# DarylFernandes99/custom-yolo-implmentation

Measured on AMD Instinct MI355X. Metric: images/sec (640x640 bf16), higher is better.
Workload: dtype bf16; 1 GPU; preset s (width 32..512, depth 1) 640x640 train step (fwd+DFL/QFL loss+bwd+grad sync+AdamW), COCO-80 synthetic, 32 img/GPU; global_batch=32, parallelism=dp1, hip_graph=True, optimizer_in_graph=True, deterministic_mode=False

## Files before the change

custom-yolo-implmentation_amd/csrc/conv_halo.hip:

```cpp
#include "conv_dev.h"

namespace {

constexpr int HROW = 48;
constexpr int HW = 18;

template <typename T, int TH, int BN, bool ACC>
__global__ __launch_bounds__((TH / 4) * (BN / 64) * 64) void k_conv_halo(GeomDev g, const T* __restrict__ src,
                                                                        const T* __restrict__ wm,
                                                                        const float* __restrict__ bias,
                                                                        T* __restrict__ dst, int tiles_h, int tiles_w,
                                                                        int ntile_n) {
    constexpr int WGM = TH / 4, WGN = BN / 64, NTHR = WGM * WGN * 64;
    constexpr int HH = TH + 2, HPX = HH * HW;
    constexpr int HR = (HPX * 4 + NTHR - 1) / NTHR;
    constexpr int WR = (BN * 4) / NTHR;
    static_assert((BN * 4) % NTHR == 0 && WR >= 1, "weight tile must divide over the workgroup");
    using ops = mfma_ops<T>;
    using frag = typename ops::frag;
    __shared__ __attribute__((aligned(16))) T halo[2][HPX * HROW];
    __shared__ __attribute__((aligned(16))) T wl[2][BN][LDSROW];

    const int tid = threadIdx.x, lane = tid & 63, wave = tid >> 6;
    const BlockTile bt = block_tile<TH, 16, BN>(tiles_h, tiles_w, ntile_n);
    const int n = bt.n, y0 = bt.y0, x0 = bt.x0, cd0 = bt.cd0;

    const int shift = (g.Ws + 1) * g.lds;
    const __amdgpu_buffer_rsrc_t rsa = __builtin_amdgcn_make_buffer_rsrc(const_cast<T*>(src) - shift, 0, (g.N * g.Hs * g.Ws * g.lds + shift) * 2, BUF_FLAGS);
    const __amdgpu_buffer_rsrc_t rsb = __builtin_amdgcn_make_buffer_rsrc(const_cast<T*>(wm), 0, g.e.Cd * g.Kpad * 2, BUF_FLAGS);
    int hvoff[HR], hlds[HR];
#pragma unroll
    for (int r = 0; r < HR; ++r) {
        const int h = tid + NTHR * r;
        const int px = h >> 2, ck = h & 3;
        const int hy = px / HW, hx = px - hy * HW;
        const bool ok = h < HPX * 4 && (unsigned)(y0 - 1 + hy) < (unsigned)g.Hs && (unsigned)(x0 - 1 + hx) < (unsigned)g.Ws;
        hvoff[r] = ok ? ((hy * g.Ws + hx) * g.lds + ck * 8) * 2 : BUF_OOB;
        hlds[r] = h < HPX * 4 ? px * HROW + ck * 8 : -1;
    }
    const int hsoff0 = (((n * g.Hs + y0 - 1) * g.Ws + x0 - 1) * g.lds + shift) * 2;
    const int kseg = tid & 3, wrow0 = tid >> 2;
    const int sk = (kseg ^ ((-(wrow0 >> 2)) & 3)) * 8;
    int wvoff[WR];
#pragma unroll
    for (int i = 0; i < WR; ++i) {
        const int row = wrow0 + i * (NTHR / 4);
        wvoff[i] = (cd0 + row < g.e.Cd) ? ((cd0 + row) * g.Kpad + kseg * 8) * 2 : BUF_OOB;
    }

    uint4 rh[HR], rw[WR];
    auto load_halo = [&](int chunk) {
#pragma unroll
        for (int r = 0; r < HR; ++r) {
            const u32x4 v = __builtin_amdgcn_raw_buffer_load_b128(rsa, hvoff[r], hsoff0 + chunk * 64, 0);
            rh[r] = make_uint4(v.x, v.y, v.z, v.w);
        }
    };
    auto store_halo = [&](int buf) {
#pragma unroll
        for (int r = 0; r < HR; ++r)
            if (hlds[r] >= 0) *reinterpret_cast<uint4*>(&halo[buf][hlds[r]]) = rh[r];
    };
    auto load_w = [&](int wcol) {
#pragma unroll
        for (int i = 0; i < WR; ++i) {
            const u32x4 v = __builtin_amdgcn_raw_buffer_load_b128(rsb, wvoff[i], wcol * 2, 0);
            rw[i] = make_uint4(v.x, v.y, v.z, v.w);
        }
    };
    auto store_w = [&](int buf) {
#pragma unroll
        for (int i = 0; i < WR; ++i) *reinterpret_cast<uint4*>(&wl[buf][wrow0 + i * (NTHR / 4)][sk]) = rw[i];
    };

    const int wgm = wave / WGN, wgn = wave - wgm * WGN;
    const int crow = wgn * 64;
    const int fr = lane & 15, fg = lane >> 4;
    const int fk = (fg ^ ((-(fr >> 2)) & 3)) * 8;
    int abase[4];
#pragma unroll
    for (int i = 0; i < 4; ++i) abase[i] = ((wgm * 4 + i + 1) * HW + fr + 1) * HROW + fg * 8;
    f32x4 acc[4][4];
#pragma unroll
    for (int i = 0; i < 4; ++i)
#pragma unroll
        for (int j = 0; j < 4; ++j) acc[i][j] = (f32x4){0.f, 0.f, 0.f, 0.f};

    const int nchunk = g.Cs / BK;
    load_halo(0);
    load_w(0);
    store_halo(0);
    store_w(0);
    __syncthreads();
    int tap = 0, chunk = 0, it = 0;
    const int nit = nchunk * g.ntaps;
    for (; it < nit; ++it) {
        const int wb = it & 1, hb = chunk & 1;
        int ntap = tap + 1, nchk = chunk;
        if (ntap == g.ntaps) { ntap = 0; ++nchk; }
        const bool more = it + 1 < nit;
        const bool new_halo = more && ntap == 0;
        if (more) load_w(ntap * g.Cs + nchk * BK);
        if (new_halo) load_halo(nchk);
        const int toff = (((int)((g.dh_pack >> (2 * tap)) & 3u) - 1) * HW + ((int)((g.dw_pack >> (2 * tap)) & 3u) - 1)) * HROW;
        frag fa[4], fb[4];
#pragma unroll
        for (int j = 0; j < 4; ++j) fa[j] = *reinterpret_cast<const frag*>(&wl[wb][crow + j * 16 + fr][fk]);
#pragma unroll
        for (int i = 0; i < 4; ++i) fb[i] = *reinterpret_cast<const frag*>(&halo[hb][abase[i] + toff]);
#pragma unroll
        for (int i = 0; i < 4; ++i)
#pragma unroll
            for (int j = 0; j < 4; ++j) acc[i][j] = ops::mma(fa[j], fb[i], acc[i][j]);
        if (more) store_w(wb ^ 1);
        if (new_halo) store_halo(hb ^ 1);
        __syncthreads();
        tap = ntap;
        chunk = nchk;
    }

    const int cq = fg * 4;
    float bv[4][4];
    bias_blocks<4>(bias, cd0 + crow, cq, g.e, bv);
    const int ox = x0 + fr;
#pragma unroll
    for (int i = 0; i < 4; ++i) {
        const int oy = y0 + wgm * 4 + i;
        const bool pv = oy < g.Hg && ox < g.Wg;
        store_pixel_blocks<T, 4, ACC>(g.e, acc[i], bv, dst, pv ? ((long)n * g.Hd + oy) * (long)g.Wd + ox : 0, pv, cd0 + crow, cq, lane);
        if (!pv) {
#pragma unroll
            for (int j = 0; j < 4; ++j) acc[i][j] = (f32x4){0.f, 0.f, 0.f, 0.f};
        }
    }

    if (g.e.stats != nullptr)
        conv_stats_epilogue<T, 4, 4>(acc, reinterpret_cast<float*>(&wl[0][0][0]), BN, g.e.stats, cd0, g.e.Cd, crow, cq, fr, tid, NTHR);
}

template <typename T, int TH, int BN>
void launch_halo(const GeomDev& d, const void* src, const void* wm, const float* bias, void* dst, int accumulate,
                 hipStream_t st) {
    constexpr int NTHR = (TH / 4) * (BN / 64) * 64;
    const int th = (d.Hg + TH - 1) / TH, tw = (d.Wg + 15) / 16, tn = (d.e.Cd + BN - 1) / BN;
    const dim3 grid((unsigned)(d.N * th * tw * tn));
    with_acc(accumulate, [&](auto acc) {
        hipLaunchKernelGGL((k_conv_halo<T, TH, BN, decltype(acc)::value>), grid, dim3(NTHR), 0, st, d, (const T*)src, (const T*)wm,
                           bias, (T*)dst, th, tw, tn);
    });
}

}

int halo_conv_eligible(const ConvGeom& g) {
    return g.sstride == 1 && g.ostep == 1 && g.ooff_h == 0 && g.ooff_w == 0 && g.ntaps > 1 && g.Cs % 32 == 0 && g.Cd >= 64 &&
           g.Hg == g.Hs && g.Wg == g.Ws && g.Hd == g.Hg && g.Wd == g.Wg;
}

int halo_conv_launch(const ConvGeom& g, int variant, const void* src, const void* wm, const float* bias, void* dst,
                     int accumulate, int dtype, hipStream_t st) {
    const GeomDev d = to_dev(g);
#define HALO_T(T_)                                                                              \
    switch (variant) {                                                                          \
        case 1: launch_halo<T_, 8, 128>(d, src, wm, bias, dst, accumulate, st); break;          \
        case 2: launch_halo<T_, 16, 128>(d, src, wm, bias, dst, accumulate, st); break;         \
        case 3: launch_halo<T_, 16, 64>(d, src, wm, bias, dst, accumulate, st); break;          \
        default: launch_halo<T_, 8, 64>(d, src, wm, bias, dst, accumulate, st); break;          \
    }
    if (dtype == YOLO_BF16) { HALO_T(bf16_t) } else { HALO_T(f16_t) }
#undef HALO_T
    return YOLO_LAUNCH_CHECK();
}
```

custom-yolo-implmentation_amd/csrc/conv_host.h:

```cpp
#pragma once
#include "common.h"
#include "conv_geom.h"

enum ConvKind {
    CONV_NONE = -1,
    CONV_VALU = 0,
    CONV_GATHER = 1,
    CONV_HALO = 2,
    CONV_RING = 3,
    CONV_ROWS = 4,
    CONV_UP2 = 5
};
struct RingTile { int bm, bn, nst, bk; };
struct ConvChoice {
    int kind;
    int joint;
    int variant;
    int bn;
    RingTile ring;
};
ConvChoice conv_select(const ConvGeom* gs, int n, int cls, int dtype, const void* src, const void* wm, const void* dst, int algo);

ConvTune& conv_tune();
int conv_wide_flag();

static inline bool desc_addressable(long elems) { return elems < (1L << 30); }
static inline bool pixels_addressable(long npix) { return npix < (1L << 31); }

int mfma_conv_addressable(const ConvGeom& g, int dtype, const void* src, const void* wm, const void* dst);

int valu_conv_launch(const ConvGeom& g, const void* src, const void* wm, const float* bias, void* dst, int accumulate, int dtype,
                     hipStream_t st);
int mfma_conv_eligible(const ConvGeom& g, int dtype, const void* src, const void* wm, const void* dst);
int mfma_conv_launch(const ConvGeom& g, int bn, const void* src, const void* wm, const float* bias, void* dst, int accumulate,
                     int dtype, hipStream_t st);
int halo_conv_eligible(const ConvGeom& g);
int halo_conv_launch(const ConvGeom& g, int variant, const void* src, const void* wm, const float* bias, void* dst,
                     int accumulate, int dtype, hipStream_t st);
int ring_conv_eligible(const ConvGeom& g, int dtype, const void* src, const void* wm, const void* dst);
int ring_conv_launch(const ConvGeom* gs, int n, const RingTile& t, const long* wm_off, long wm_elems, const void* src,
                     const void* wm, const float* bias, void* dst, int accumulate, int dtype, hipStream_t st);
int rows_conv_eligible(const ConvGeom& g);
int rows_conv_launch(const ConvGeom& g, int variant, const void* src, const void* wm, const float* bias, void* dst, int accumulate,
                     int dtype, hipStream_t st);
int up2_conv_eligible(const ConvGeom* gs, int dtype);
int up2_conv_launch(const ConvGeom* gs, int variant, const long* wm_off, long wm_elems, const void* src, const void* wm, void* dst,
                    int accumulate, int dtype, hipStream_t st);
int f32_conv_eligible(const ConvGeom& g, const void* src, const void* wm, const void* dst);
int f32_conv_launch(const ConvGeom& g, const float* src, const float* wm, const float* bias, float* dst, int accumulate,
                    hipStream_t st);

int f32_wgrad_eligible(const void* x, int ldx, const void* dy, int ldy, int Cin, int Cout);
int f32_wgrad_launch(const float* x, int ldx, const float* dy, int ldy, float* dwp, int Kpad, int N, int H, int W, int Cin,
                     int OH, int OW, int Cout, int k, int stride, hipStream_t st);
int mfma_wgrad_eligible(int Cin, int Cout, int ldx, int ldy, int dtype, const void* x, const void* dy);
int mfma_wgrad_launch(const void* x, int ldx, const void* dy, int ldy, float* dwp, int Kpad, int N, int H, int W,
                      int Cin, int OH, int OW, int Cout, int k, int stride, int dtype, hipStream_t st);
long mfma_wgrad2_plan(int Kpad, int N, int H, int W, int Cin, int OH, int OW, int Cout, int k);
long mfma_wgrad2_ws_elems(int Kpad, int N, int H, int W, int Cin, int OH, int OW, int Cout, int k);
int mfma_wgrad2_launch(const void* x, int ldx, const void* dy, int ldy, float* part, void* dw_oihw, int dw_dtype, int Kpad,
                       int N, int H, int W, int Cin, int OH, int OW, int Cout, int k, int stride, int dtype, hipStream_t st);

struct DwPlan {
    int cvb, ncy;
    int ncol, ncb;
    int wg;
    int hb, nb, grid;
    int hb_wg, nb_wg, grid_wg;
};
DwPlan dw_plan(int N, int H, int W, int C);
int dw_tune_set(int variant);
bool dw_takes_rows(int N, int H, int W, int C, bool wgrad);
int dw16_launch(bool flip, const void* x, int ldx, const float* w, void* y, int ldy, int N, int H, int W, int C, int dtype,
                int accumulate, float* stats, hipStream_t st, const float* bias = nullptr, int act = 0);
int dw16_wgrad_launch(const void* x, int ldx, const void* dy, int ldy, float* partial, int nslab, int* nrows, int N, int H, int W,
                      int C, int dtype, hipStream_t st);

extern "C" int yolo_bn_stats_acc(const void* y, int ldy, long npix, int C, int dtype, float* acc, hipStream_t st);
extern "C" int yolo_copy_channels(const void* src, int ld_src, void* dst, int ld_dst, long npix, int C, int accumulate, int dtype,
                                  hipStream_t st);

static inline bool conv_supported(int k, int stride) { return (k == 1 && stride == 1) || (k == 3 && (stride == 1 || stride == 2)); }
static inline bool conv_supported(int k, int stride, int Cin, int Cout) {
    return conv_supported(k, stride) && Cin >= 0 && Cout >= 0 && (long)k * k * (Cin > Cout ? Cin : Cout) <= 2147483647L - 31;
}
```

custom-yolo-implmentation_amd/csrc/conv_rows.hip:

```cpp
#include "conv_dev.h"

namespace {

template <typename T, int W, int WGM, int NWAVE, int WN, int NST, bool ACC>
__global__ __launch_bounds__(64 * NWAVE) void k_conv_rows(GeomDev g, const T* __restrict__ src, const T* __restrict__ wm,
                                                   const float* __restrict__ bias, T* __restrict__ dst, int tiles_h,
                                                   int tiles_w, int ntile_n) {
    constexpr int R = WGM * 80 / W, HWID = W == 16 ? 18 : W + 8, HH = R + 2, HPX = HH * HWID;
    constexpr int WGN = NWAVE / WGM;
    constexpr int NTHR = 64 * NWAVE, BN = WGN * WN * 16;
    constexpr int HP = ((HPX + 15) / 16 + NWAVE - 1) / NWAVE;
    constexpr int DW = (3 * BN / 16 + NWAVE - 1) / NWAVE;
    constexpr int HBUF = NWAVE * HP * 1024, STAGE = NWAVE * DW * 1024;
    static_assert(R * W == WGM * 80 && NST >= 3 && NST <= 4 && NWAVE == 4, "block shape");
    using ops = mfma_ops<T>;
    using frag = typename ops::frag;
    extern __shared__ __attribute__((aligned(1024))) char rows_smem[];
    const unsigned lds0 = __builtin_amdgcn_readfirstlane((unsigned)(size_t)(__attribute__((address_space(3))) char*)rows_smem);

    const int tid = threadIdx.x, lane = tid & 63, wave = __builtin_amdgcn_readfirstlane(tid >> 6);
    const BlockTile bt = block_tile<R, W, BN>(tiles_h, tiles_w, ntile_n);
    const int n = bt.n, y0 = bt.y0, x0 = bt.x0, cd0 = bt.cd0;

    const int shift = (g.Ws + 1) * g.lds;
    const int a_bytes = (g.N * g.Hs * g.Ws * g.lds + shift) * 2, w_bytes = g.e.Cd * g.Kpad * 2;
    int hvoff[HP], wvoff[DW];
#pragma unroll
    for (int i = 0; i < HP; ++i) {
        const int px = (wave * HP + i) * 16 + (lane >> 2), ck = (lane & 3) ^ ((px >> 1) & 3);
        const int hy = px / HWID, hx = px - hy * HWID;
        const bool ok = px < HPX && (unsigned)(y0 - 1 + hy) < (unsigned)g.Hs && (unsigned)(x0 + hx - 1) < (unsigned)g.Ws;
        hvoff[i] = (ok && ck * 8 < g.Cs) ? ((hy * g.Ws + hx) * g.lds + ck * 8) * 2 : BUF_OOB;
    }
    const int hsoff0 = (((n * g.Hs + y0 - 1) * g.Ws + x0 - 1) * g.lds + shift) * 2;
#pragma unroll
    for (int j = 0; j < DW; ++j) {
        const int rs = (wave * DW + j) * 16 + (lane >> 2);
        const int tl = rs / BN, row = rs - tl * BN;
        const int kseg = (lane & 3) ^ ((-(row >> 2)) & 3);
        wvoff[j] = (tl < 3 && cd0 + row < g.e.Cd && kseg * 8 < g.Cs) ? ((cd0 + row) * g.Kpad + tl * g.Cs + kseg * 8) * 2 : BUF_OOB;
    }
    const int nchunk = (g.Cs + BK - 1) / BK, nit = nchunk * 3;
    auto issue_halo = [&](int chunk) {
        const __amdgpu_buffer_rsrc_t rsa = __builtin_amdgcn_make_buffer_rsrc(const_cast<T*>(src) - shift, 0, chunk < nchunk ? a_bytes : 0, BUF_FLAGS);
        const unsigned base = lds0 + (chunk & 1) * HBUF + wave * (HP * 1024);
#pragma unroll
        for (int i = 0; i < HP; ++i) lds_dma_piece(rsa, base + i * 1024, hvoff[i], hsoff0 + chunk * 64);
    };
    int wstep = 0, wchunk = 0, wrow = 0, wbuf = 0;
    auto issue_w = [&]() {
        const __amdgpu_buffer_rsrc_t rsb = __builtin_amdgcn_make_buffer_rsrc(const_cast<T*>(wm), 0, wstep < nit ? w_bytes : 0, BUF_FLAGS);
        const unsigned base = lds0 + 2 * HBUF + wbuf * STAGE + wave * (DW * 1024);
        const int soff = (3 * wrow * g.Cs + wchunk * BK) * 2;
#pragma unroll
        for (int j = 0; j < DW; ++j) lds_dma_piece(rsb, base + j * 1024, wvoff[j], soff);
        ++wstep;
        if (++wrow == 3) { wrow = 0; ++wchunk; }
        if (++wbuf == NST) wbuf = 0;
    };

    const int wgm = wave / WGN, wgn = wave - wgm * WGN;
    const int crow = wgn * WN * 16;
    const int fr = lane & 15, fg = lane >> 4;
    const int fk = (fg ^ ((-(fr >> 2)) & 3)) * 16;
    int aoff[5][9];
#pragma unroll
    for (int i = 0; i < 5; ++i) {
        const int p = (wgm * 5 + i) * 16 + fr, pr = p / W, pc = p - pr * W;
#pragma unroll
        for (int tap = 0; tap < 9; ++tap) {
            const int px = (pr + (int)((g.dh_pack >> (2 * tap)) & 3u)) * HWID + pc + (int)((g.dw_pack >> (2 * tap)) & 3u);
            aoff[i][tap] = px * 64 + ((fg ^ ((px >> 1) & 3)) << 4);
        }
    }
    const int woff = (crow + fr) * 64 + fk;
    f32x4 acc[5][WN];
#pragma unroll
    for (int i = 0; i < 5; ++i)
#pragma unroll
        for (int j = 0; j < WN; ++j) acc[i][j] = (f32x4){0.f, 0.f, 0.f, 0.f};

    issue_halo(0);
#pragma unroll
    for (int s = 0; s < NST - 1; ++s) issue_w();
    int rbuf = 0;
    auto step = [&](auto srow_c, auto par_c, int chunk) {
        constexpr int srow = decltype(srow_c)::value, par = decltype(par_c)::value;
        constexpr bool patch_newer = srow != 0 && (NST == 4 || srow == 1);
        dma_wait<(NST - 2) * DW + (patch_newer ? HP : 0)>();
        __builtin_amdgcn_s_barrier();
        if (srow == 0) issue_halo(chunk + 1);
        issue_w();
        const char* hp = rows_smem + par * HBUF;
        const char* wp = rows_smem + 2 * HBUF + (NST == 3 ? srow : rbuf) * STAGE;
#pragma unroll
        for (int tl = 0; tl < 3; ++tl) {
            const int tap = 3 * srow + tl;
            frag fa[WN], fb[5];
#pragma unroll
            for (int j = 0; j < WN; ++j) fa[j] = *reinterpret_cast<const frag*>(wp + (tl * BN + j * 16) * 64 + woff);
#pragma unroll
            for (int i = 0; i < 5; ++i) fb[i] = *reinterpret_cast<const frag*>(hp + aoff[i][tap]);
#pragma unroll
            for (int i = 0; i < 5; ++i)
#pragma unroll
                for (int j = 0; j < WN; ++j) acc[i][j] = ops::mma(fa[j], fb[i], acc[i][j]);
        }
        if (++rbuf == NST) rbuf = 0;
    };
    using c0 = ic<0>; using c1 = ic<1>; using c2 = ic<2>;
    int chunk = 0;
    for (; chunk + 1 < nchunk; chunk += 2) {
        step(c0{}, c0{}, chunk); step(c1{}, c0{}, chunk); step(c2{}, c0{}, chunk);
        step(c0{}, c1{}, chunk + 1); step(c1{}, c1{}, chunk + 1); step(c2{}, c1{}, chunk + 1);
    }
    if (chunk < nchunk) { step(c0{}, c0{}, chunk); step(c1{}, c0{}, chunk); step(c2{}, c0{}, chunk); }
    dma_wait<0>();
    __syncthreads();

    const int cq = fg * 4;
    float bv[WN][4];
    bias_blocks<WN>(bias, cd0 + crow, cq, g.e, bv);
#pragma unroll
    for (int i = 0; i < 5; ++i) {
        const int p = (wgm * 5 + i) * 16 + fr, pr = p / W, pc = p - pr * W;
        const int oy = y0 + pr, ox = x0 + pc;
        const bool live = oy < g.Hg && ox < g.Wg;
        store_pixel_blocks<T, WN, ACC>(g.e, acc[i], bv, dst, live ? ((long)n * g.Hd + oy) * (long)g.Wd + ox : 0, live, cd0 + crow, cq, lane);
        if (!live) {
#pragma unroll
            for (int j = 0; j < WN; ++j) acc[i][j] = (f32x4){0.f, 0.f, 0.f, 0.f};
        }
    }

    if (g.e.stats != nullptr)
        conv_stats_epilogue<T, 5, WN>(acc, reinterpret_cast<float*>(rows_smem), BN, g.e.stats, cd0, g.e.Cd, crow, cq, fr, tid, NTHR);
}

template <typename T, int W, int WGM, int NWAVE, int WN, int NST>
int launch_rows(const GeomDev& d, const void* src, const void* wm, const float* bias, void* dst, int accumulate, hipStream_t st) {
    constexpr int R = WGM * 80 / W, BN = (NWAVE / WGM) * WN * 16, HPX = (R + 2) * (W == 16 ? 18 : W + 8);
    constexpr size_t lds = 2 * (size_t)(NWAVE * (((HPX + 15) / 16 + NWAVE - 1) / NWAVE)) * 1024 + (size_t)NST * NWAVE * ((3 * BN / 16 + NWAVE - 1) / NWAVE) * 1024;
    const int th = (d.Hg + R - 1) / R, tw = W == 16 ? (d.Wg + 15) / 16 : 1, tn = (d.e.Cd + BN - 1) / BN;
    const dim3 grid((unsigned)(d.N * th * tw * tn));
    return with_acc(accumulate, [&](auto acc) {
        return launch_dyn_lds<k_conv_rows<T, W, WGM, NWAVE, WN, NST, decltype(acc)::value>>(grid, dim3(64 * NWAVE), lds, st, d, (const T*)src,
                                                                                            (const T*)wm, bias, (T*)dst, th, tw, tn);
    });
}

}

int rows_conv_eligible(const ConvGeom& g) {
    if (!(g.sstride == 1 && g.ostep == 1 && g.ooff_h == 0 && g.ooff_w == 0 && g.ntaps == 9 && (g.Cs % 32 == 0 || g.Cs == 16) && g.Cd >= 16 &&
          g.Cd % 8 == 0 && g.Hg == g.Hs && g.Wg == g.Ws && g.Hd == g.Hg && g.Wd == g.Wg))
        return 0;
    for (int t = 0; t < 9; ++t)
        if (g.dh[t] < -1 || g.dh[t] > 1 || g.dw[t] < -1 || g.dw[t] > 1) return 0;
    if (g.Cd < 64 || g.Cs == 16) return 3;
    return (g.Wg == 20 || g.Wg == 40) ? 1 : 2;
}

int rows_conv_launch(const ConvGeom& g, int variant, const void* src, const void* wm, const float* bias, void* dst, int accumulate,
                     int dtype, hipStream_t st) {
    const GeomDev d = to_dev(g);
#define ROWS_W(T_, W_)                                                                                               \
    switch (variant) {                                                                                               \
        case 2: return launch_rows<T_, W_, 1, 4, 2, 3>(d, src, wm, bias, dst, accumulate, st);                          \
        case 3: return launch_rows<T_, W_, 1, 4, 1, 3>(d, src, wm, bias, dst, accumulate, st);                       \
        case 4: return launch_rows<T_, W_, 2, 4, 2, 3>(d, src, wm, bias, dst, accumulate, st);                       \
        default: return launch_rows<T_, W_, 1, 4, 1, 4>(d, src, wm, bias, dst, accumulate, st);                         \
    }
#define ROWS_T(T_)                                                                                                   \
    if (variant == 6) return launch_rows<T_, 16, 2, 4, 2, 3>(d, src, wm, bias, dst, accumulate, st);    \
    if (variant == 7) return launch_rows<T_, 16, 4, 4, 2, 3>(d, src, wm, bias, dst, accumulate, st);    \
    if (g.Wg == 20) { ROWS_W(T_, 20) }                                                                               \
    ROWS_W(T_, 40)
    if (dtype == YOLO_BF16) { ROWS_T(bf16_t) }
    ROWS_T(f16_t)
#undef ROWS_T
#undef ROWS_W
}
```

include/yolo_hip.h:

```cpp
#ifndef YOLO_HIP_H
#define YOLO_HIP_H
#include <stddef.h>
#include <stdint.h>

#ifdef __cplusplus
extern "C" {
#endif

#ifndef __HIP__
typedef struct ihipStream_t* hipStream_t;
#endif

#define YOLO_F32 0
#define YOLO_BF16 1
#define YOLO_F16 2
#define YOLO_ERR_ARG 1001
#define YOLO_ERR_DTYPE 1002
#define YOLO_ACT_IDENTITY 0
#define YOLO_ACT_SILU 1

long yolo_abi_hash(void);

int yolo_memset0(void* p, size_t bytes, hipStream_t st);
int yolo_ncm_to_nhwc(const void* src, int src_dtype, long sn, long sc, long off, void* dst, int dst_dtype, int ld, int N, int C, int HW, hipStream_t st);
int yolo_nhwc_to_ncm(const void* src, int src_dtype, int ld, void* dst, int dst_dtype, long sn, long sc, long off, int N, int C, int HW, hipStream_t st);
int yolo_head_group(int pack, int n, void* const* branches, const int* lds, const int* Cs, const int* HWs, const int* c_offs, const int* m_offs, void* preds, int cp, int M, int N, int dtype, hipStream_t st);
int yolo_copy_channels(const void* src, int ld_src, void* dst, int ld_dst, long npix, int C, int accumulate, int dtype, hipStream_t st);
int yolo_scale_inplace(void* x, long n, int dtype, const float* scale_dev, hipStream_t st);
int yolo_add_n(const void* s0, int ld0, const void* s1, int ld1, const void* s2, int ld2, const void* s3, int ld3, int nsrc, void* dst, int ld_dst, long npix, int C, int dtype, hipStream_t st);

int yolo_conv_kpad(int O, int I, int k, int stride, int mode, int cls);
long yolo_conv_dgrad_wbuf_elems(int O, int I, int k, int stride);
int yolo_conv_pack_weights(const void* w_oihw, int w_dtype, int O, int I, int k, int stride, int mode, void* out, int out_dtype, hipStream_t st);
int yolo_conv_unpack_wgrad(const float* dwp, int O, int I, int k, void* dw_oihw, int dw_dtype, hipStream_t st);
int yolo_pack_job_bytes();
int yolo_pack_job_count(int stride, int mode);
long yolo_pack_job_fill(void* jobs_host, const void* w, int w_dtype, void* out, int out_elem_bytes, int O, int I, int k, int stride, int mode, long start);
long yolo_pack_jobs_finalize(void* jobs_host, int njobs);
int yolo_pack_batched(const void* jobs_dev, int njobs, long nchunks, int out_dtype, hipStream_t st);
int yolo_adamw_job_bytes();
int yolo_adamw_job_fill(void* jobs_host, int index, void* p, int p_dtype, const void* g, int g_dtype, float* m, float* v, long n);
long yolo_adamw_jobs_finalize(void* jobs_host, int njobs);
int yolo_adamw_jobs_set_grads(void* jobs_host, int njobs, const void* const* grads);
int yolo_adamw_step(const void* jobs_dev, int njobs, long nchunks, const double* hyper, float* step, const float* grad_scale, const float* found_inf, hipStream_t st);
int yolo_adamw_job_set_ema(void* jobs_host, int index, float* ema, double* ema_ctl);
int yolo_ema_lerp(const void* jobs_dev, int njobs, long nchunks, const double* ema_ctl, const float* skip_flag, hipStream_t st);
int yolo_adamw_amp_step(const void* jobs_dev, int njobs, long nchunks, const double* hyper, float* step, float* amp_state, int* growth_tracker, float growth_factor, float backoff_factor, int growth_interval, hipStream_t st);
int yolo_grad_sqnorm(const void* jobs_dev, int njobs, long nchunks, float* partials, float* found_inf, hipStream_t st);
int yolo_grad_clip_finalize(const float* partials, long nparts, float* clip_state, const float* grad_scale, hipStream_t st);
int yolo_adamw_clip_step(const void* jobs_dev, int njobs, long nchunks, const double* hyper, float* step, const float* grad_scale, const float* found_inf, const float* clip_state, hipStream_t st);
int yolo_amp_update_scale(float* amp_state, int* growth_tracker, float growth_factor, float backoff_factor, int growth_interval, hipStream_t st);
int yolo_sgd_step(const void* jobs_dev, int njobs, long nchunks, const double* hyper, float* step, const float* grad_scale, const float* found_inf, const float* clip_state, hipStream_t st);
int yolo_sgd_amp_step(const void* jobs_dev, int njobs, long nchunks, const double* hyper, float* step, float* amp_state, int* growth_tracker, float growth_factor, float backoff_factor, int growth_interval, hipStream_t st);
int yolo_copy_job_bytes();
int yolo_copy_job_fill(void* jobs_host, int index, const void* src, int src_dtype, void* dst, int dst_dtype, long n);
long yolo_copy_jobs_finalize(void* jobs_host, int njobs);
int yolo_multi_copy(const void* jobs_dev, int njobs, long nchunks, float scale, hipStream_t st);
int yolo_conv2d_fwd(const void* x, int ldx, const void* wp, const float* bias, void* y, int ldy, float* stats_acc, int N, int H, int W, int Cin, int OH, int OW, int Cout, int k, int stride, int dtype, int algo, hipStream_t st);
int yolo_conv2d_fwd_act(const void* x, int ldx, const void* wp, const float* bias, const void* res, int ldr, void* y, int ldy, int N, int H, int W, int Cin, int OH, int OW, int Cout, int k, int stride, int act, int dtype, hipStream_t st);
int yolo_conv2d_dgrad(const void* dy, int lddy, const void* wb, void* dx, int lddx, int N, int H, int W, int Cin, int OH, int OW, int Cout, int k, int stride, int accumulate, int dtype, int algo, hipStream_t st);
int yolo_conv2d_dgrad_acc2(const void* dy, int lddy, const void* wb, void* dx, int lddx, const void* acc2, int ld2, int N, int H, int W, int Cin, int OH, int OW, int Cout, int k, int stride, int dtype, int algo, hipStream_t st);
long yolo_conv2d_wgrad_ws_elems(const void* x, int ldx, const void* dy, int ldy, int N, int H, int W, int Cin, int OH, int OW, int Cout, int k, int stride, int dtype, int algo);
int yolo_conv2d_wgrad(const void* x, int ldx, const void* dy, int ldy, float* ws, void* dw_oihw, int dw_dtype, int N, int H, int W, int Cin, int OH, int OW, int Cout, int k, int stride, int dtype, int algo, hipStream_t st);
int yolo_conv_tune_set(int bn, int tap_inner, int halo, int dma, int ring, int bm, int nst, int bk);
int yolo_wgrad_tune_set(int to, int ti, int blocks, int min_per);
int yolo_wgrad_tune_pf(int pf);
int yolo_conv_wide_set(int on);
int yolo_conv2d_plan(int N, int H, int W, int Cin, int OH, int OW, int Cout, int k, int stride, int mode, int cls, int dtype);
long yolo_conv2d_wgrad_plan(int N, int H, int W, int Cin, int OH, int OW, int Cout, int k, int stride, int dtype);
int yolo_stem_im2col(const void* img, int img_dtype, void* col, int col_dtype, int N, int H, int W, int OH, int OW, hipStream_t st);
int yolo_stem_pack_weights(const void* w, int w_dtype, int Cout, void* out, int out_dtype, hipStream_t st);
int yolo_stem_unpack_wgrad(const float* dw32, int Cout, void* dw, int dw_dtype, hipStream_t st);
int yolo_stem_conv_eligible(int img_dtype, int dtype, int Cout);
int yolo_stem_conv_fwd(const float* img, const void* wp, void* y, int ldy, float* stats, int N, int H, int W, int OH, int OW, int Cout, const float* bias, int act, int dtype, hipStream_t st);
int yolo_stem_wgrad_slabs();
int yolo_stem_wgrad(const float* img, const void* dy, int ldy, float* partial, void* dw, int dw_dtype, int N, int H, int W, int OH, int OW, int Cout, int dtype, hipStream_t st);
long yolo_stem_bn_wgrad_ws_elems(int Cout);
int yolo_stem_bn_wgrad(const float* img, const void* dout, int ldd, const void* y, int ldy, const float* scale, const float* shift, const void* gamma, const float* mean, const float* invstd, float* partial, void* dw, int dw_dtype, void* dgamma, void* dbeta, int N, int H, int W, int OH, int OW, int Cout, int act, int dtype, int pdt, hipStream_t st);
int yolo_dwconv3x3_fwd(const void* x, int ldx, const float* w, void* y, int ldy, int N, int H, int W, int C, int dtype, hipStream_t st);
int yolo_dwconv3x3_fwd_stats(const void* x, int ldx, const float* w, void* y, int ldy, float* stats, int N, int H, int W, int C, int dtype, hipStream_t st);
int yolo_dwconv3x3_fwd_act(const void* x, int ldx, const float* w, const float* bias, void* y, int ldy, int N, int H, int W, int C, int act, int dtype, hipStream_t st);
int yolo_dwconv3x3_dgrad(const void* dy, int lddy, const float* w, void* dx, int lddx, int N, int H, int W, int C, int accumulate, int dtype, hipStream_t st);
int yolo_dw_wgrad_nslab(int N, int H);
int yolo_dwconv3x3_wgrad(const void* x, int ldx, const void* dy, int ldy, float* dw, float* partial, int N, int H, int W, int C, int dtype, hipStream_t st);
int yolo_dw_tune_set(int variant);
int yolo_dw_plan(int N, int H, int W, int C, int field);

int yolo_reduce_nblk(long npix, int C);
int yolo_bn_stats(const void* y, int ldy, long npix, int C, int dtype, float* partial, int nblk, hipStream_t st);
int yolo_bn_finalize(const float* partial, int nblk, long count, int C, const void* gamma, const void* beta, void* running_mean, void* running_var, float momentum, float eps, float* mean, float* invstd, float* scale, float* shift, int pdtype, int bdtype, hipStream_t st);
int yolo_bn_eval_coeffs(const void* gamma, const void* beta, const void* running_mean, const void* running_var, float eps, int C, float* scale, float* shift, int pdtype, int bdtype, hipStream_t st);
int yolo_sum_finalize(const float* partial, int nblk, int C, float* out, hipStream_t st);
int yolo_bn_act_fwd(const void* y, int ldy, const float* scale, const float* shift, const void* res, int ldres, void* out, int ldout, long npix, int C, int act, int dtype, hipStream_t st);
int yolo_bn_act_bwd_reduce(const void* dout, int ldd, const void* y, int ldy, const float* scale, const float* shift, const float* mean, const float* invstd, long npix, int C, int act, int dtype, float* partial, int nblk, hipStream_t st);
int yolo_bn_bwd_finalize(const float* partial, int nblk, long count, int C, const void* gamma, const float* mean, const float* invstd, void* dgamma, void* dbeta, float* coef, int pdtype, hipStream_t st);
int yolo_bn_act_bwd_apply(const void* dout, int ldd, const void* y, int ldy, const float* scale, const float* shift, const float* mean, const float* invstd, const float* coef, void* dy, int lddy, long npix, int C, int act, int dtype, hipStream_t st);
int yolo_bn_acc_elems(int C);
int yolo_bn_stats_acc(const void* y, int ldy, long npix, int C, int dtype, float* acc, hipStream_t st);
int yolo_bn_finalize_acc(const float* acc, long count, int C, const void* gamma, const void* beta, void* running_mean, void* running_var, float momentum, float eps, float* mean, float* invstd, float* scale, float* shift, int pdtype, int bdtype, hipStream_t st);
int yolo_bn_act_fwd_train(const void* y, int ldy, const float* acc, long count, const void* gamma, const void* beta, void* running_mean, void* running_var, float momentum, float eps, float* mean, float* invstd, float* scale, float* shift, const void* res, int ldres, void* out, int ldout, long npix, int C, int act, int dtype, int pdtype, int bdtype, hipStream_t st);
int yolo_bn_bwd_reduce_acc(const void* dout, int ldd, const void* y, int ldy, const float* scale, const float* shift, long npix, int C, int act, int dtype, float* acc, hipStream_t st);
int yolo_bn_act_bwd_apply_train(const void* dout, int ldd, const void* y, int ldy, const float* scale, const float* shift, const void* gamma, const float* mean, const float* invstd, const float* acc, long count, void* dgamma, void* dbeta, void* dy, int lddy, long npix, int C, int act, int dtype, int pdtype, hipStream_t st);

int yolo_maxpool5_fwd(const void* x, int ldx, void* out, int ldo, uint8_t* idx, int N, int H, int W, int C, int dtype, hipStream_t st);
int yolo_maxpool5_bwd(const void* dout, int ldd, const uint8_t* idx, void* dx, int ldx, int N, int H, int W, int C, int accumulate, int dtype, hipStream_t st);
int yolo_upsample2x_fwd(const void* x, int ldx, void* out, int ldo, int N, int H, int W, int C, int dtype, hipStream_t st);
int yolo_upsample2x_bwd(const void* dout, int ldd, void* dx, int ldx, int N, int H, int W, int C, int accumulate, int dtype, hipStream_t st);

size_t yolo_attn_stash_bytes(int N, int T_, int heads, int dtype);
size_t yolo_attn_workspace_bytes(int N, int T_, int heads, int dtype);
size_t yolo_attn_stash_bytes_for(int N, int T, int heads, int dk, int dh, int dtype);
size_t yolo_attn_workspace_bytes_for(int N, int T, int heads, int dk, int dh, int dtype);
int yolo_attn_fwd(const void* qkv, int ldq, void* o, int ldo, void* vp, int ldv, void* stash, void* ws, int N, int T_, int heads, int dk, int dh, float scale, int dtype, hipStream_t st);
int yolo_attn_fwd_nograd(const void* qkv, int ldq, void* o, int ldo, void* vp, int ldv, int N, int T_, int heads, int dk, int dh, float scale, int dtype, hipStream_t st);
int yolo_attn_bwd(const void* qkv, int ldq, const void* o, int ldo, const void* d_o, int lddo, const void* d_vp, int lddv, const void* stash, void* ws, void* dqkv, int lddq, int N, int T_, int heads, int dk, int dh, float scale, int dtype, hipStream_t st);

size_t yolo_loss_workspace_bytes(int N, int A, int G);
int yolo_loss_dfl_qfl(const void* preds, const void* anchors, const void* strides, int dtype, int N, int nc, int A, const float* gt, const int* gt_off, const int* gt_img, int G, float lambda_dfl, float lambda_cls, void* dpreds, float* out, void* workspace, const float* grad_scale, hipStream_t st);

size_t yolo_loss_tal_workspace_bytes(int N, int A, int G);
int yolo_loss_tal(const void* preds, const void* anchors, const void* strides, int dtype, int N, int nc, int A, const float* gt, const int* gt_off, const int* gt_img, int G, int topk, float alpha, float beta, float lambda_box, float lambda_cls, float lambda_dfl, void* dpreds, float* out, void* workspace, const float* grad_scale, hipStream_t st);

int yolo_bbox_iou(const float* box1, const float* box2, int M, float* iou, const float* g, float* db1, float* db2, hipStream_t st);
int yolo_quality_focal_loss(const float* pred, const float* target, int M, int C, float beta, float* out, const float* g, float* dpred, float* dtarget, hipStream_t st);
int yolo_distribution_focal_loss(const float* pred_dist, const float* target_val, int M, int C, float* out, const float* g, float* dpred, float* dtarget, hipStream_t st);

int yolo_head_decode(const void* preds, const void* anchors, const void* strides, void* y, int N, int nc, int A, int dtype, hipStream_t st);
int yolo_dfl_expect(const void* x, void* y, int B, int A, int dtype, hipStream_t st);
int yolo_nms_capacity(int M, int nc, int multi_label);
size_t yolo_nms_workspace_bytes(int bs, int M, int nc, int multi_label);
int yolo_nms(const void* y, int dtype, int bs, int nc, int M, float conf_thres, float iou_thres, const int* classes, int n_classes, int agnostic, int multi_label, int max_det, float* out, int* out_count, int* status, void* workspace, hipStream_t st);
int yolo_rows_to_source(float* rows, const int* counts, const void* table_dev, int N, int max_det, int prob, hipStream_t st);

size_t yolo_val_workspace_bytes(int N, int M, int top_k);
int yolo_val_select(const void* y, int dtype, int N, int nc, int M, float conf, int top_k, float* out, int* out_count, void* workspace, hipStream_t st);
int yolo_val_match(const float* pred, const int* count, int N, int top_k, const float* gt, const int* gt_off, double iou_thr, int nc, int skip_empty_gt, long long* counters, int* status, hipStream_t st);

int yolo_ap_match(const float* det, const int* count, int N, int K, const float* gt, const int* gt_off, const double* iou_thr, int n_thr, int nc, long long* key, unsigned* tp, long long* gt_count, int* status, hipStream_t st);
int yolo_ap_curve(const long long* key, const unsigned* tp, long D, const long long* gt_count, const double* rec_thr, int nc, int n_thr, double* precision, hipStream_t st);

int yolo_prep_image_bytes();
int yolo_prep_image_fill(void* table_host, int index, long off, int H, int W, int flip, int o0, int o1, int o2, int o3, float brightness, float contrast, float saturation, float hue);
int yolo_image_prep(const void* src, const void* table_dev, int N, int S, int jitter, void* stage, float* means, void* out, int out_dtype, float m0, float m1, float m2, float s0, float s1, float s2, hipStream_t st);
int yolo_mosaic_tile_bytes();
int yolo_mosaic_tile_fill(void* table_host, int image, int tile, long off, int H, int W, int flip, int tw, int th, int x0, int y0, int cx, int cy);
int yolo_image_prep_mosaic(const void* src, const void* tiles_dev, const void* table_dev, int N, int S, int fill, int jitter, void* stage, float* means, void* out, int out_dtype, float m0, float m1, float m2, float s0, float s1, float s2, hipStream_t st);
int yolo_affine_bytes();
int yolo_affine_fill(void* table_host, int index, float a00, float a01, float b0, float a10, float a11, float b1);
int yolo_image_prep_affine(const void* src, const void* tiles_dev, const void* table_dev, const void* affine_dev, int N, int S, int fill, int jitter, void* stage, void* stage2, float* means, void* out, int out_dtype, float m0, float m1, float m2, float s0, float s1, float s2, hipStream_t st);
int yolo_mix_bytes();
int yolo_mix_fill(void* table_host, int index, int partner, float r, int N);
int yolo_image_prep_mixup(const void* src, const void* tiles_dev, const void* table_dev, const void* affine_dev, const void* mix_dev, int N, int S, int fill, int jitter, void* stage, void* stage2, float* means, void* out, int out_dtype, float m0, float m1, float m2, float s0, float s1, float s2, hipStream_t st);
int yolo_letter_bytes();
int yolo_letter_fill(void* table_host, int index, long off, int H, int W, int nw, int nh, int left, int top, float sx, float sy, int S, long src_bytes);
int yolo_letterbox(const void* src, const void* table_dev, int N, int S, int fill, void* out, int out_dtype, float m0, float m1, float m2, float s0, float s1, float s2, hipStream_t st);

int yolo_selftest_tr16(const void* tile_in, void* out, hipStream_t st);
int yolo_selftest_glds(const void* in128x16, void* out64x16, hipStream_t st);
int yolo_selftest_dma_vs_xlane(const void* pattern4k, int blocks, int iters, int spam, void* errors, void* sink, hipStream_t st);
int yolo_selftest_dma_order(const void* src, long src_bytes, int blocks, int kind, void* errors2, hipStream_t st);
int yolo_selftest_ring_vs_xlane(const void* src, int steps, int blocks, int spam, void* errors, void* sink, hipStream_t st);
int yolo_selftest_permlane16(const void* in64, void* out128, hipStream_t st);
int yolo_selftest_grid_barrier(void* counters, int blocks, int rounds, int tree, int* timed_out, hipStream_t st);

#ifdef __cplusplus
}
#endif
#endif
```

Baseline: 3141 images/s.

## Add row-streaming 3x3 conv kernel with register-resident weights for narrow channels

Adds a new 3x3 stride-1 convolution kernel for small channel counts (Cs, Cd ≤ 64) on large feature maps. Each workgroup keeps all of its weights in registers and streams input rows through an LDS ring buffer using DMA, processing a vertical band of the image so that each row is loaded once and reused across all three vertical taps. The halo and rows paths hand off to this kernel when the geometry qualifies. The aim is to cut the repeated halo reloads and weight LDS traffic of the existing tiled kernels on the high-resolution, low-channel layers. In exchange it raises register pressure and can lower occupancy.

Result: no change. 3171 images/s (median of 6 runs) (+1.0%).

```diff
diff --git a/custom-yolo-implmentation_amd/csrc/conv_halo.hip b/custom-yolo-implmentation_amd/csrc/conv_halo.hip
--- a/custom-yolo-implmentation_amd/csrc/conv_halo.hip
+++ b/custom-yolo-implmentation_amd/csrc/conv_halo.hip
@@ -159,8 +159,9 @@
 
 int halo_conv_launch(const ConvGeom& g, int variant, const void* src, const void* wm, const float* bias, void* dst,
                      int accumulate, int dtype, hipStream_t st) {
+    if (stream_conv_takes(g, dtype, src, wm, dst)) return stream_conv_launch(g, src, wm, bias, dst, accumulate, dtype, st);
     const GeomDev d = to_dev(g);
-#define HALO_T(T_)                                                                              \
+#define HALO_T(T_)                                                                             \
     switch (variant) {                                                                          \
         case 1: launch_halo<T_, 8, 128>(d, src, wm, bias, dst, accumulate, st); break;          \
         case 2: launch_halo<T_, 16, 128>(d, src, wm, bias, dst, accumulate, st); break;         \
diff --git a/custom-yolo-implmentation_amd/csrc/conv_host.h b/custom-yolo-implmentation_amd/csrc/conv_host.h
--- a/custom-yolo-implmentation_amd/csrc/conv_host.h
+++ b/custom-yolo-implmentation_amd/csrc/conv_host.h
@@ -43,6 +43,9 @@
 int rows_conv_eligible(const ConvGeom& g);
 int rows_conv_launch(const ConvGeom& g, int variant, const void* src, const void* wm, const float* bias, void* dst, int accumulate,
                      int dtype, hipStream_t st);
+int stream_conv_takes(const ConvGeom& g, int dtype, const void* src, const void* wm, const void* dst);
+int stream_conv_launch(const ConvGeom& g, const void* src, const void* wm, const float* bias, void* dst, int accumulate, int dtype,
+                       hipStream_t st);
 int up2_conv_eligible(const ConvGeom* gs, int dtype);
 int up2_conv_launch(const ConvGeom* gs, int variant, const long* wm_off, long wm_elems, const void* src, const void* wm, void* dst,
                     int accumulate, int dtype, hipStream_t st);
diff --git a/custom-yolo-implmentation_amd/csrc/conv_rows.hip b/custom-yolo-implmentation_amd/csrc/conv_rows.hip
--- a/custom-yolo-implmentation_amd/csrc/conv_rows.hip
+++ b/custom-yolo-implmentation_amd/csrc/conv_rows.hip
@@ -163,6 +163,8 @@
 
 int rows_conv_launch(const ConvGeom& g, int variant, const void* src, const void* wm, const float* bias, void* dst, int accumulate,
                      int dtype, hipStream_t st) {
+    if ((variant == 6 || variant == 7) && stream_conv_takes(g, dtype, src, wm, dst))
+        return stream_conv_launch(g, src, wm, bias, dst, accumulate, dtype, st);
     const GeomDev d = to_dev(g);
 #define ROWS_W(T_, W_)                                                                                               \
     switch (variant) {                                                                                               \
diff --git a/custom-yolo-implmentation_amd/csrc/conv_stream.hip b/custom-yolo-implmentation_amd/csrc/conv_stream.hip
--- /dev/null
+++ b/custom-yolo-implmentation_amd/csrc/conv_stream.hip
@@ -0,0 +1,320 @@
+#include <cstdlib>
+#include "conv_dev.h"
+
+namespace {
+
+constexpr int ST_LDS_CU = 160 * 1024;
+constexpr int ST_CUS = 256;
+constexpr int ST_MIN_BAND = 28;
+
+template <int NCH, int WGM> struct StreamCfg {
+    static constexpr int WGN = 4 / WGM;
+    static constexpr int RW = 2;
+    static constexpr int RS = RW * WGM;
+    static constexpr int P = 4 / WGM;
+    static constexpr int NSLOT = (P + 1) * RS + 2;
+    static constexpr int ENT = 18 * NCH;
+    static constexpr int PPR = (ENT + 15) / 16;
+    static constexpr int SLOTB = PPR * 1024;
+    static constexpr int PW = (RS / 4) * PPR;
+    static constexpr int BN = WGN * 32;
+    static constexpr int LDS = NSLOT * SLOTB;
+};
+
+template <typename T, int NCH, int WGM, bool ACC>
+__global__ __launch_bounds__(256, NCH <= 2 ? 2 : 1)
+void k_conv_stream(GeomDev g, const T* __restrict__ src, const T* __restrict__ wm, const float* __restrict__ bias,
+                   T* __restrict__ dst, int hb, int nb, int tiles_w, int ntile_n) {
+    using C = StreamCfg<NCH, WGM>;
+    constexpr int WGN = C::WGN, RW = C::RW, RS = C::RS, P = C::P, NSLOT = C::NSLOT, ENT = C::ENT, PPR = C::PPR, SLOTB = C::SLOTB;
+    constexpr int PW = C::PW, BN = C::BN, NTHR = 256;
+    using ops = mfma_ops<T>;
+    using frag = typename ops::frag;
+    extern __shared__ __attribute__((aligned(1024))) char stream_smem[];
+    const unsigned lds0 = __builtin_amdgcn_readfirstlane((unsigned)(size_t)(__attribute__((address_space(3))) char*)stream_smem);
+
+    const int tid = threadIdx.x, lane = tid & 63, wave = __builtin_amdgcn_readfirstlane(tid >> 6);
+    int t = xcd_remap(blockIdx.x, gridDim.x);
+    const int tile_n = t % ntile_n; t /= ntile_n;
+    const int band = t % nb; t /= nb;
+    const int tx = t % tiles_w, n = t / tiles_w;
+    const int x0 = tx * 16, yb = band * hb, cd0 = tile_n * BN;
+    const int hbe = (g.Hg - yb) < hb ? (g.Hg - yb) : hb;
+    const int nstep = (hbe + RS - 1) / RS;
+
+    const int shift = g.lds;
+    const int a_bytes = (g.N * g.Hs * g.Ws * g.lds + shift) * 2;
+    int hvoff[PPR];
+#pragma unroll
+    for (int p = 0; p < PPR; ++p) {
+        const int e = p * 16 + (lane >> 2), c = e / 18, px = e - c * 18, ck = (lane & 3) ^ ((e >> 1) & 3);
+        const bool ok = e < ENT && (unsigned)(x0 - 1 + px) < (unsigned)g.Ws;
+        hvoff[p] = ok ? (px * g.lds + c * 32 + ck * 8) * 2 : BUF_OOB;
+    }
+    auto issue_row = [&](int q) {
+        const int r = yb - 1 + q;
+        const bool ok = (unsigned)r < (unsigned)g.Hs && q <= hbe + 1;
+        const __amdgpu_buffer_rsrc_t rsa = __builtin_amdgcn_make_buffer_rsrc(const_cast<T*>(src) - shift, 0, ok ? a_bytes : 0, BUF_FLAGS);
+        const int soff = ok ? (((n * g.Hs + r) * g.Ws + x0 - 1) * g.lds + shift) * 2 : 0;
+        const unsigned base = lds0 + ((unsigned)q % (unsigned)NSLOT) * SLOTB;
+#pragma unroll
+        for (int p = 0; p < PPR; ++p) lds_dma_piece(rsa, base + p * 1024, hvoff[p], soff);
+    };
+    auto issue_batch = [&](int b) {
+#pragma unroll
+        for (int k = 0; k < RS / 4; ++k) issue_row(2 + b * RS + wave + 4 * k);
+    };
+    if (wave < 2) issue_row(wave);
+#pragma unroll
+    for (int b = 0; b < P; ++b) issue_batch(b);
+
+    const int wgm = wave / WGN, wgn = wave - wgm * WGN;
+    const int crow = wgn * 32;
+    const int fr = lane & 15, fg = lane >> 4;
+    frag wr[NCH][9][2];
+    {
+        const __amdgpu_buffer_rsrc_t rsb = __builtin_amdgcn_make_buffer_rsrc(const_cast<T*>(wm), 0, g.e.Cd * g.Kpad * 2, BUF_FLAGS);
+        int wvoff[2];
+#pragma unroll
+        for (int j = 0; j < 2; ++j) {
+            const int row = cd0 + crow + j * 16 + fr;
+            wvoff[j] = row < g.e.Cd ? (row * g.Kpad + fg * 8) * 2 : BUF_OOB;
+        }
+#pragma unroll
+        for (int c = 0; c < NCH; ++c)
+#pragma unroll
+            for (int tap = 0; tap < 9; ++tap)
+#pragma unroll
+                for (int j = 0; j < 2; ++j) {
+                    const u32x4 v = __builtin_amdgcn_raw_buffer_load_b128(rsb, wvoff[j], (tap * g.Cs + c * 32) * 2, 0);
+                    wr[c][tap][j] = __builtin_bit_cast(frag, v);
+                }
+    }
+    int loff[NCH][3];
+#pragma unroll
+    for (int c = 0; c < NCH; ++c)
+#pragma unroll
+        for (int d = 0; d < 3; ++d) {
+            const int e = c * 18 + fr + d;
+            loff[c][d] = e * 64 + ((fg ^ ((e >> 1) & 3)) << 4);
+        }
+    const int cq = fg * 4;
+    float bv[2][4];
+    bias_blocks<2>(bias, cd0 + crow, cq, g.e, bv);
+    const int ox = x0 + fr, yend = yb + hbe;
+    const bool want_stats = g.e.stats != nullptr;
+    float ssum[2][4], ssq[2][4];
+#pragma unroll
+    for (int j = 0; j < 2; ++j)
+#pragma unroll
+        for (int r = 0; r < 4; ++r) ssum[j][r] = ssq[j][r] = 0.f;
+
+    for (int s = 0; s < nstep; ++s) {
+        dma_wait<(P - 1) * PW>();
+        __builtin_amdgcn_s_barrier();
+        issue_batch(s + P);
+        const int wq = s * RS + wgm * RW;
+        f32x4 acc[RW][2];
+#pragma unroll
+        for (int i = 0; i < RW; ++i)
+#pragma unroll
+            for (int j = 0; j < 2; ++j) acc[i][j] = (f32x4){0.f, 0.f, 0.f, 0.f};
+#pragma unroll
+        for (int c = 0; c < NCH; ++c) {
+            frag fb[RW + 2][3];
+#pragma unroll
+            for (int k = 0; k < RW + 2; ++k) {
+                const char* rp = stream_smem + ((unsigned)(wq + k) % (unsigned)NSLOT) * SLOTB;
+#pragma unroll
+                for (int d = 0; d < 3; ++d) fb[k][d] = *reinterpret_cast<const frag*>(rp + loff[c][d]);
+            }
+#pragma unroll
+            for (int tap = 0; tap < 9; ++tap)
+#pragma unroll
+                for (int i = 0; i < RW; ++i)
+#pragma unroll
+                    for (int j = 0; j < 2; ++j) acc[i][j] = ops::mma(wr[c][tap][j], fb[i + tap / 3][tap % 3], acc[i][j]);
+        }
+#pragma unroll
+        for (int i = 0; i < RW; ++i) {
+            const int oy = yb + wq + i;
+            const bool live = oy < yend && ox < g.Wg;
+            store_pixel_blocks<T, 2, ACC>(g.e, acc[i], bv, dst, live ? ((long)n * g.Hd + oy) * (long)g.Wd + ox : 0, live, cd0 + crow, cq, lane);
+            if (want_stats && live) {
+#pragma unroll
+                for (int j = 0; j < 2; ++j)
+#pragma unroll
+                    for (int r = 0; r < 4; ++r) {
+                        const float v = to_f<T>(from_f<T>(acc[i][j][r]));
+                        ssum[j][r] += v;
+                        ssq[j][r] += v * v;
+                    }
+            }
+        }
+    }
+    dma_wait<0>();
+    __syncthreads();
+
+    if (want_stats) {
+        float* sacc = reinterpret_cast<float*>(stream_smem);
+        stats_zero(sacc, 2 * BN, tid, NTHR);
+        __syncthreads();
+#pragma unroll
+        for (int j = 0; j < 2; ++j)
+#pragma unroll
+            for (int r = 0; r < 4; ++r) {
+                const float s1 = row16_sum(ssum[j][r]), s2 = row16_sum(ssq[j][r]);
+                if (fr == 0) {
+                    atomicAdd(&sacc[crow + j * 16 + cq + r], s1);
+                    atomicAdd(&sacc[BN + crow + j * 16 + cq + r], s2);
+                }
+            }
+        __syncthreads();
+        stats_flush(sacc, BN, g.e.stats, cd0, g.e.Cd, tid, NTHR);
+    }
+}
+
+int& stream_mode() {
+    static int v = [] {
+        const char* e = getenv("YOLO_CONV_STREAM");
+        return e == nullptr ? 1 : (atoi(e) != 0 ? 1 : 0);
+    }();
+    return v;
+}
+
+struct StreamPlan {
+    int fits;
+    int nch, wgm, bn, rs, nslot, lds;
+    int tw, tn;
+    int hb, nb, grid;
+    int cap;
+};
+
+template <int NCH, int WGM> void plan_cfg(StreamPlan& p) {
+    using C = StreamCfg<NCH, WGM>;
+    p.bn = C::BN; p.rs = C::RS; p.nslot = C::NSLOT; p.lds = C::LDS;
+}
+
+StreamPlan stream_plan(long N, long H, long W, long Cs, long Cd) {
+    StreamPlan p{};
+    if (N <= 0 || H <= 0 || W <= 0 || Cs < 32 || Cs > 128 || Cs % 32 || Cd < 8 || Cd % 8) return p;
+    p.nch = (int)(Cs / 32);
+    p.wgm = Cd <= 32 ? 4 : 2;
+    switch (p.nch * 10 + p.wgm) {
+        case 12: plan_cfg<1, 2>(p); break;
+        case 14: plan_cfg<1, 4>(p); break;
+        case 22: plan_cfg<2, 2>(p); break;
+        case 24: plan_cfg<2, 4>(p); break;
+        case 32: plan_cfg<3, 2>(p); break;
+        case 34: plan_cfg<3, 4>(p); break;
+        case 42: plan_cfg<4, 2>(p); break;
+        default: plan_cfg<4, 4>(p); break;
+    }
+    int per_cu = ST_LDS_CU / p.lds;
+    if (per_cu < 1) return p;
+    const int by_regs = p.nch == 1 ? 4 : p.nch == 2 ? 2 : 1;
+    if (per_cu > by_regs) per_cu = by_regs;
+    p.cap = ST_CUS * per_cu;
+    const long tw = (W + 15) / 16, tn = (Cd + p.bn - 1) / p.bn;
+    const long per_band = N * tw * tn;
+    if (per_band > 0x7fffffffL) return p;
+    const long want = p.cap / per_band > 1 ? p.cap / per_band : 1;
+    long hb = (H + want - 1) / want;
+    if (hb < ST_MIN_BAND) hb = ST_MIN_BAND;
+    hb = (hb + p.rs - 1) / p.rs * p.rs;
+    const long nb = (H + hb - 1) / hb;
+    if (per_band * nb > 0x7fffffffL) return p;
+    p.tw = (int)tw; p.tn = (int)tn; p.hb = (int)hb; p.nb = (int)nb; p.grid = (int)(per_band * nb);
+    p.fits = 1;
+    return p;
+}
+
+bool stream_measured(const ConvGeom& g) {
+    if (g.Cs > 64 || g.Cd > 64 || g.Hg < 80 || g.Wg < 80) return false;
+    return stream_plan(g.N, g.Hg, g.Wg, g.Cs, g.Cd).grid >= ST_CUS;
+}
+
+template <typename T, int NCH, int WGM>
+int launch_stream(const GeomDev& d, const StreamPlan& p, const void* src, const void* wm, const float* bias, void* dst, int accumulate,
+                  hipStream_t st) {
+    return with_acc(accumulate, [&](auto acc) {
+        return launch_dyn_lds<k_conv_stream<T, NCH, WGM, decltype(acc)::value>>(dim3((unsigned)p.grid), dim3(256), (size_t)p.lds, st, d,
+                                                                                (const T*)src, (const T*)wm, bias, (T*)dst, p.hb, p.nb,
+                                                                                p.tw, p.tn);
+    });
+}
+
+}
+
+int stream_conv_takes(const ConvGeom& g, int dtype, const void* src, const void* wm, const void* dst) {
+    const int mode = stream_mode();
+    if (mode == 0) return 0;
+    if (dtype != YOLO_BF16 && dtype != YOLO_F16) return 0;
+    if (!(g.sstride == 1 && g.ostep == 1 && g.ooff_h == 0 && g.ooff_w == 0 && g.ntaps == 9 && g.Hg == g.Hs && g.Wg == g.Ws &&
+          g.Hd == g.Hg && g.Wd == g.Wg && g.Kpad == 9 * g.Cs))
+        return 0;
+    for (int t = 0; t < 9; ++t)
+        if (g.dh[t] != t / 3 - 1 || g.dw[t] != t % 3 - 1) return 0;
+    if (!stream_plan(g.N, g.Hg, g.Wg, g.Cs, g.Cd).fits) return 0;
+    if (g.lds % 8 || g.ldd % 4 || g.lds < g.Cs || (reinterpret_cast<uintptr_t>(src) & 15) || (reinterpret_cast<uintptr_t>(wm) & 15) ||
+        (reinterpret_cast<uintptr_t>(dst) & 7))
+        return 0;
+    if (!desc_addressable((long)g.N * g.Hs * g.Ws * g.lds + g.lds) || !desc_addressable((long)g.Cd * g.Kpad) ||
+        !pixels_addressable((long)g.N * g.Hd * g.Wd))
+        return 0;
+    return mode == 2 || stream_measured(g);
+}
+
+int stream_conv_launch(const ConvGeom& g, const void* src, const void* wm, const float* bias, void* dst, int accumulate, int dtype,
+                       hipStream_t st) {
+    const GeomDev d = to_dev(g);
+    const StreamPlan p = stream_plan(g.N, g.Hg, g.Wg, g.Cs, g.Cd);
+    if (!p.fits) return YOLO_ERR_ARG;
+#define STREAM_C(T_, NCH_)                                                                        \
+    case NCH_: return p.wgm == 2 ? launch_stream<T_, NCH_, 2>(d, p, src, wm, bias, dst, accumulate, st) \
+                                 : launch_stream<T_, NCH_, 4>(d, p, src, wm, bias, dst, accumulate, st);
+#define STREAM_T(T_)                                                                              \
+    switch (p.nch) { STREAM_C(T_, 1) STREAM_C(T_, 2) STREAM_C(T_, 3) STREAM_C(T_, 4) default: return YOLO_ERR_ARG; }
+    if (dtype == YOLO_BF16) { STREAM_T(bf16_t) }
+    STREAM_T(f16_t)
+#undef STREAM_T
+#undef STREAM_C
+}
+
+extern "C" {
+
+int yolo_conv_stream_set(int mode) {
+    if (mode < 0 || mode > 2) return YOLO_ERR_ARG;
+    stream_mode() = mode;
+    return YOLO_OK;
+}
+
+int yolo_conv_stream_plan(int N, int H, int W, int Cs, int Cd, int dtype, int field) {
+    const StreamPlan p = stream_plan(N, H, W, Cs, Cd);
+    if (field == 0) {
+        if (N <= 0 || H <= 0 || W <= 0 || Cs <= 0 || Cd <= 0 || (long)9 * Cs > 2147483647L - 31) return 0;
+        ConvGeom g{};
+        g.N = N; g.Hs = g.Hd = g.Hg = H; g.Ws = g.Wd = g.Wg = W; g.Cs = Cs; g.lds = Cs; g.Cd = Cd; g.ldd = Cd;
+        g.ostep = 1; g.sstride = 1; g.ntaps = 9;
+        for (int t = 0; t < 9; ++t) { g.dh[t] = t / 3 - 1; g.dw[t] = t % 3 - 1; }
+        g.K = 9 * Cs; g.Kpad = round_up32(g.K);
+        alignas(16) static const char nominal[16] = {};
+        return stream_conv_takes(g, dtype, nominal, nominal, nominal);
+    }
+    switch (field) {
+        case 1: return p.fits;
+        case 2: return p.hb;
+        case 3: return p.nb;
+        case 4: return p.grid;
+        case 5: return p.lds;
+        case 6: return p.bn;
+        case 7: return p.rs;
+        case 8: return p.nslot;
+        case 9: return p.cap;
+        case 10: return p.tw;
+        case 11: return p.tn;
+        default: return -1;
+    }
+}
+
+}
diff --git a/include/yolo_hip.h b/include/yolo_hip.h
--- a/include/yolo_hip.h
+++ b/include/yolo_hip.h
@@ -67,6 +67,8 @@
 int yolo_wgrad_tune_pf(int pf);
 int yolo_conv_wide_set(int on);
 int yolo_conv2d_plan(int N, int H, int W, int Cin, int OH, int OW, int Cout, int k, int stride, int mode, int cls, int dtype);
+int yolo_conv_stream_set(int mode);
+int yolo_conv_stream_plan(int N, int H, int W, int Cs, int Cd, int dtype, int field);
 long yolo_conv2d_wgrad_plan(int N, int H, int W, int Cin, int OH, int OW, int Cout, int k, int stride, int dtype);
 int yolo_stem_im2col(const void* img, int img_dtype, void* col, int col_dtype, int N, int H, int W, int OH, int OW, hipStream_t st);
 int yolo_stem_pack_weights(const void* w, int w_dtype, int Cout, void* out, int out_dtype, hipStream_t st);
```
